# uuwee/Vulkan-PBR-Renderer

Hardware: AMD Instinct MI355X
Metric: IBL-prefilter Mtexels/s (specular prefilter all mips + irradiance; PBR-shaded Mpixels/s under extra.shade_c5 / extra.shade) (higher is better)
Workload: dtype f32; 1 GPU; C4: 4096x4096 specular prefilter (6 faces, 13 mips) + 128x128 irradiance from a 2048^2 HDR cube; env=procedural HDR cube 2048^2 x6 RGBA32F (seed 0x5eed0004, RGBE round-tripped), overlap=False, parallelism=single GPU

## Files before the change

include/pbr_kernels.h:

```cpp
#ifndef PBR_KERNELS_H
#define PBR_KERNELS_H

#include <stddef.h>
#include <stdint.h>

#ifdef __cplusplus
extern "C" {
#endif

enum {
    PBRK_OK = 0,
    PBRK_E_ARG = -1,
    PBRK_E_FORMAT = -2,
    PBRK_E_LAUNCH = -3
};

enum {
    PBRK_FMT_RG16F = 1,
    PBRK_FMT_RG32F = 2,
    PBRK_FMT_RGBA16F = 3,
    PBRK_FMT_RGBA32F = 4,
    PBRK_FMT_R32F = 5,
    PBRK_FMT_RGBA8UN = 6,
    PBRK_FMT_BGRA8UN = 7
// ... 41 lines not shown
size_t pbrk_cells_bytes(int n_src);
int pbrk_cells_build(const void* bordered_level, int n_src, void* cells, void* stream);
int pbrk_mc_filter(const void* src_bordered_level, const void* src_cells, int n_src, const void* table4, int n_entries,
                   float divisor, float alpha, void* out, int out_size,
                   int face0, int face1, int y0, int y1, void* stream);

int pbrk_mc_region_stats(unsigned long long* out2, int reset);
void pbrk_mc_set_kernels(int region, int lds);
int pbrk_mc_region_flag_stats(unsigned long long* out3);
int pbrk_mc_region_window_stats(unsigned long long* out1);
int pbrk_mc_region_skip_stats(unsigned long long* out3);
void pbrk_mc_set_absorb(int on);
void pbrk_mc_set_runs(int on);
void pbrk_mc_set_prologue(int lean);
int pbrk_mc_region_phase_stats(unsigned long long* out5);
int pbrk_mc_region_order(int face, int G, int k);
void pbrk_mc_set_launch_cut(int on);
int pbrk_mc_launch_cut(const float* weights, int n, unsigned min_bits, unsigned max_bits, int* cut4);
int pbrk_mc_launch_cut_slices(const float* weights, int n, int S, unsigned min_bits, unsigned max_bits, int* cut);
int pbrk_mc_launch_cut_stats(int* out6);
void pbrk_mc_set_tile32(int mode);
void pbrk_mc_set_fold(int on);
int pbrk_mc_last_fold(void);
void pbrk_mc_set_resident(int on);
int pbrk_mc_resident_stats(unsigned long long* out4);

typedef struct PbrkShadeArgs {
    int width, height;
    int x0, x1, y0, y1;
    const void* base_color;
    const void* normal;
    const void* orm;
    const void* emissive;
    const void* depth;
    const void* irradiance_bordered;
    int irradiance_size;
    const void* prefiltered_bordered;
    int prefiltered_size, prefiltered_levels;
    const void* lut;
    int lut_size;
    const void* irradiance_cells;
    const void* prefiltered_cells;
    int prefiltered_cells_first;
    const void* lut_cells;
    const void* sun_depth;
    int sun_depth_w, sun_depth_h;
// ... 150 lines not shown
```

vulkan-pbr-renderer_amd/csrc/k_mc_internal.h:

```cpp
#pragma once
#include <hip/hip_runtime.h>
#include "pbr_device.h"

struct McArgs {
    const float4* src; int n_src; unsigned src_bytes;
    const float4* cells; unsigned cells_bytes;
    const float4* tab; int n_tab;
    float divisor, alpha;
    float4* out; int size;
    int face0, y0, rows, tiles_x, tiles_per_face;
    int snap;
};

typedef unsigned int u32x3 __attribute__((ext_vector_type(3)));


__device__ __forceinline__ f3 tap_rgb(__amdgpu_buffer_rsrc_t rs, int voff, int soff) {
    u32x3 v = __builtin_amdgcn_raw_buffer_load_b96(rs, voff, soff, 0);
    return mk3(__uint_as_float(v.x), __uint_as_float(v.y), __uint_as_float(v.z));
}

typedef unsigned int u32x4c __attribute__((ext_vector_type(4)));
__device__ __forceinline__ f3 fetch_cells(__amdgpu_buffer_rsrc_t rc, int voff, float a, float b) {
    u32x4c A = __builtin_amdgcn_raw_buffer_load_b128(rc, voff, 0, 0);
// ... 44 lines not shown
    union { unsigned u; float f; } cm, cM, cW;
    cm.u = min_bits; cM.u = max_bits;
    const double m = (double)cm.f, M = (double)cM.f;
    int ncut = 0;
    for (int s = 0; s < S; ++s) {
        const double rhs = H[s] * m;
        if (!(rhs * 0x1p-25 >= 0x1p-100)) continue;
        int c = cut[s];
        for (int w = c - S; w > s; w -= S) {
            cW.u = wbits[w];
            const double lhs = (double)cW.f * M * 0x1p25 * (1.0 + 0x1p-10);
            if (!(lhs <= rhs)) break;
            c = w;
        }
        ncut += (cut[s] - c) / S;
        cut[s] = c;
    }
    return ncut;
}
__host__ __device__ inline int mc_launch_cut(const unsigned* wbits, int NW, const double* H, unsigned min_bits, unsigned max_bits, int* cut4) {
    return mc_launch_cut_s(wbits, NW, 4, H, min_bits, max_bits, cut4);
}

bool launch_mc_region(McArgs a, int nfaces, hipStream_t st);
bool launch_mc_resident(McArgs a, int nfaces, hipStream_t st);
extern int g_mc_region_mode, g_mc_lds_mode;
```

vulkan-pbr-renderer_amd/csrc/k_mc_region.hip:

```cpp
#include "pbr_device.h"
#include "pbr_kernels.h"
#include "k_mc_internal.h"

#include <stdlib.h>
#include <mutex>
#include <type_traits>

typedef float v4f __attribute__((ext_vector_type(4)));
typedef const __attribute__((address_space(4))) v4f* ctab_t;
typedef const __attribute__((address_space(3))) v4f* lds_v4f_p;
typedef const __attribute__((address_space(4))) unsigned* cu32_t;

#define REG_MAX_S 16
#ifndef MC_HEAD_FIRST_SUB
#define MC_HEAD_FIRST_SUB 1
#endif
#ifndef MC_HEAD_FIRST_G1
#define MC_HEAD_FIRST_G1 1
#endif
#ifndef MC_CERT_G1
#define MC_CERT_G1 1
#endif

#ifndef MC_TAP_JOIN_G1
#define MC_TAP_JOIN_G1 1
#endif

#ifndef MC_TILE32_SUB
#define MC_TILE32_SUB 1
#endif
#ifndef MC_TILE32_MIN_SIZE
#define MC_TILE32_MIN_SIZE 1024
#endif

struct RegArgs {
    McArgs a;
    int G;
    int RC;
    int NR;
    int NW;
    int expect[REG_MAX_S];
    int pole_row[2];
    const unsigned* tabmax;
    int cut;
    int absorb;
    unsigned long long* stats;
};

__device__ __forceinline__ void face_coords(int f, float x, float y, float z, float& sc, float& tc, float& ma) {
    switch (f) {
    case 0: sc = -z; tc = -y; ma = x; break;
    case 1: sc = z; tc = -y; ma = -x; break;
// ... 56 lines not shown
    unsigned long long inm = __builtin_amdgcn_ballot_w64(c1) & __builtin_amdgcn_ballot_w64(c2);
    if (inm == 0) return;
    if (!ACC && !SUB) { cnt += (unsigned)__builtin_popcountll(inm); return; }
    bool in = c1 && c2;
    const float h = __builtin_amdgcn_rcpf(ma) * V.half_n;
    const float u = fmaf(sc, h, V.off), v = fmaf(tc, h, V.off);
    if (SUB) {
        const bool c3 = u >= V.ulo, c4 = u < V.uhi, c5 = v >= V.vlo, c6 = v < V.vhi;
        inm &= __builtin_amdgcn_ballot_w64(c3) & __builtin_amdgcn_ballot_w64(c4) & __builtin_amdgcn_ballot_w64(c5) & __builtin_amdgcn_ballot_w64(c6);
        in = in && c3 && c4 && c5 && c6;
    }
    cnt += (unsigned)__builtin_popcountll(inm);
    if (ACC && in) tap_accumulate<RS>(e.w, u, v, V.lds_base, ar, ag, ab);
}

template <int RS, bool FOLD = false, bool JOIN = false>
__device__ __forceinline__ void certain_sample(const v4f e, const RegionView& V, float& ar, float& ag, float& ab) {
    float sc, tc, ma;
    to_face(e, V, sc, tc, ma);
    const float h = FOLD ? __builtin_amdgcn_rcpf(ma) : __builtin_amdgcn_rcpf(ma) * V.half_n;
    tap_accumulate<RS, JOIN>(e.w, fmaf(sc, h, V.off), fmaf(tc, h, V.off), V.lds_base, ar, ag, ab);
}

template <int RS, bool SUB, int CLS, bool ACC = true, bool FOLD = false, bool JOIN = false>
__device__ __forceinline__ void lane_sample(const v4f e, const RegionView& V, float& ar, float& ag, float& ab, unsigned& cnt) {
    float sc, tc, ma;
    to_face(e, V, sc, tc, ma);
    bool c1, c2;
    on_face<CLS>(sc, tc, FOLD ? ma * V.half_n : ma, c1, c2);
    bool in = c1 && c2;
    if (SUB && __builtin_amdgcn_ballot_w64(in) == 0ull) return;
    const float h = FOLD ? __builtin_amdgcn_rcpf(ma) : __builtin_amdgcn_rcpf(ma) * V.half_n;
    const float u = fmaf(sc, h, V.off), v = fmaf(tc, h, V.off);
    if (SUB) in = in && u >= V.ulo && u < V.uhi && v >= V.vlo && v < V.vhi;
    if (in) {
        cnt += 1u;
        if (ACC) tap_accumulate<RS, JOIN>(e.w, u, v, V.lds_base, ar, ag, ab);
    }
}

template <typename F>
__device__ __forceinline__ void each_sample(unsigned m, ctab_t tw, F&& f) {
    if (m == 0u) return;
    v4f e = tw[__builtin_ctz(m)];
    m &= m - 1u;
    while (m) {
        const v4f en = tw[__builtin_ctz(m)];
        m &= m - 1u;
        f(e);
        e = en;
    }
    f(e);
}

__device__ __forceinline__ float absorb_threshold(float wmax, float m) {
    const float t = wmax * m * 1.00000095367431640625f * 0x1p25f;
    return t < 0x1p-100f ? 0x1p-100f : t;
}

// ... 36 lines not shown
                    region_sample<RS, SUB, CLS, false>(tw[i0], V, ar, ag, ab, cnt);
                }
                continue;
            }
        }
        while (m) {
            const int i0 = __builtin_ctz(m);
            m &= m - 1u;
            const bool two = m != 0u;
            const int i1 = two ? __builtin_ctz(m) : i0;
            m &= m - 1u;
            const v4f e0 = tw[i0];
            const v4f e1 = tw[i1];
            if (CERT && ((c >> i0) & 1u)) certain_sample<RS>(e0, V, ar, ag, ab);
            else region_sample<RS, SUB, CLS>(e0, V, ar, ag, ab, cnt);
            if (two) {
                if (CERT && ((c >> i1) & 1u)) certain_sample<RS>(e1, V, ar, ag, ab);
                else region_sample<RS, SUB, CLS>(e1, V, ar, ag, ab, cnt);
            }
        }
    }
}

template <int RS, bool SUB, int CLS, int REG_S, bool CERT, bool LEAN, bool FOLD>
__device__ __forceinline__ void region_pass_runs(const RegionView& V, const unsigned* __restrict__ mwords, const unsigned* __restrict__ cwords, cu32_t wmg,
                                                 unsigned rbits, unsigned* skc, int NW, int s, unsigned long long wsel, ctab_t tab,
                                                 float& ar, float& ag, float& ab, unsigned& cnt) {
    const int wl = s + REG_S * (int)(threadIdx.x & 63);
    unsigned long long nz = __builtin_amdgcn_ballot_w64(wl < NW && mwords[wl] != 0u) & wsel;
    constexpr bool JOIN = FOLD && RS == 66 && !SUB && MC_TAP_JOIN_G1 != 0;
    auto tested = [&](const v4f e) { lane_sample<RS, SUB, CLS, true, FOLD, JOIN>(e, V, ar, ag, ab, cnt); };
    while (nz) {
        const int w = s + REG_S * (int)__builtin_ctzll(nz);
        nz &= nz - 1ull;
        const unsigned m = (unsigned)__builtin_amdgcn_readfirstlane((int)mwords[w]);
        unsigned c = CERT ? (unsigned)__builtin_amdgcn_readfirstlane((int)cwords[w]) : 0u;
        ctab_t tw = tab + (w << 5);
        const unsigned wb = rbits < 0x7f800000u ? (LEAN ? wmg[w] : (unsigned)__builtin_amdgcn_readfirstlane((int)cwords[NW + w])) : 0x7f800000u;
        if (wb < 0x7f800000u) {
            const float T = absorb_threshold(__uint_as_float(wb), __uint_as_float(rbits));
            if (__builtin_amdgcn_ballot_w64(!(ar >= T && ag >= T && ab >= T)) == 0ull) {
                if (!CERT) c = (unsigned)__builtin_amdgcn_readfirstlane((int)cwords[w]);
                cnt += (unsigned)__builtin_popcount(m & c);
                count_absorbed(skc, m, m & ~c);
                each_sample(m & ~c, tw, [&](const v4f e) { lane_sample<RS, SUB, CLS, false, FOLD>(e, V, ar, ag, ab, cnt); });
                continue;
            }
        }
        if (!CERT) { each_sample(m, tw, tested); continue; }
        cnt += (unsigned)__builtin_popcount(m & c);
        unsigned mc = m & c, mu = m & ~c;
        for (;;) {
            const unsigned below = mu ? (mu & (0u - mu)) - 1u : ~0u;
            each_sample(mc & below, tw, [&](const v4f e) { certain_sample<RS, FOLD, JOIN>(e, V, ar, ag, ab); });
            mc &= ~below;
            if (!mu) break;
            const int it = __builtin_ctz(mu);
            mu &= mu - 1u;
            tested(tw[it]);
        }
    }
}

template <bool LEAN, bool G1, bool TWO, bool PROOF, bool SOLE>
__device__ __forceinline__ void region_bin(unsigned* masks, unsigned* any, unsigned* dmax, int NR, int NW, int G, int RC, int n,
                                           f3 R, f3 T, f3 B, f3 Rc, f3 Tc, f3 Bc, ctab_t tab, int n_tab, int tid,
                                           unsigned* cmask, unsigned* wmax, int ntail, int lim, bool keep_cut, int head_end) {
    const float nf = (float)n;
    const float half_n = 0.5f * nf;
    const float off = 0.5f * nf + 0.5f;
    for (int k = tid; k < NR * NW + NR + 1 + ntail; k += 1024) masks[k] = 0u;
    __syncthreads();
    {
// ... 162 lines not shown
template <int REG_TX, int REG_S>
__device__ __forceinline__ void reduce_slices(float* red, int s, int t, float ar, float ag, float ab) {
    red[(s * REG_TX + t) * 3 + 0] = ar;
    red[(s * REG_TX + t) * 3 + 1] = ag;
    red[(s * REG_TX + t) * 3 + 2] = ab;
    __syncthreads();
    for (int stride = REG_S / 2; stride >= 1; stride >>= 1) {
        if (s < stride) {
            const int a2 = (s * REG_TX + t) * 3, b2 = ((s + stride) * REG_TX + t) * 3;
            red[a2 + 0] += red[b2 + 0];
            red[a2 + 1] += red[b2 + 1];
            red[a2 + 2] += red[b2 + 2];
        }
        __syncthreads();
    }
}

#ifdef PBR_MC_PHASE_STAMPS
#define STAMP() ((unsigned long long)__builtin_readcyclecounter())
#else
#define STAMP() 0ull
#endif

template <int RS, bool SUB, int TILE, bool RUNS = false, bool LEAN = false, bool FOLD = false>
__global__ __launch_bounds__(1024) __attribute__((amdgpu_waves_per_eu(8, 8))) void k_mc_region(const RegArgs q) {
    constexpr int REG_TX = TILE * TILE, REG_S = 1024 / REG_TX;
    static_assert(!FOLD || (RUNS && LEAN && RS != 18), "FOLD: the run loop of the lean 66^2 / 34^2 shapes only");
    constexpr bool CERT = SUB || (RUNS && (RS != 66 || MC_CERT_G1 != 0));
    constexpr bool ABS = RS == 66;
    const bool absorb_on = ABS && q.absorb;
    constexpr bool OWN_FIRST = ABS;
    constexpr bool TWO = RS == 66 && (SUB ? MC_HEAD_FIRST_SUB != 0 : MC_HEAD_FIRST_G1 != 0);
    const bool cut_on = TWO && LEAN && q.cut != 0;
    extern __shared__ __attribute__((aligned(16))) unsigned char smem_r[];
    float4* region = (float4*)smem_r;
    const unsigned lds_base = (unsigned)(unsigned long long)smem_r;
    unsigned* skc = (unsigned*)(smem_r + RS * RS * 16);
    unsigned* masks = skc + 4;
    unsigned* any = masks + q.NR * q.NW;
    unsigned* dmax = any + q.NR;
    unsigned* cmask = dmax + 1;
    unsigned* wmax = cmask + q.NW;
    unsigned* rmax = wmax + q.NW;
    const int ntail = (absorb_on && !LEAN) ? 2 * q.NW + q.NR : ((CERT || ABS) ? q.NW : 0);
    cu32_t wmg = (cu32_t)(unsigned long long)q.tabmax;
    [[maybe_unused]] const unsigned long long st0 = STAMP();
    const McArgs& p = q.a;
    const int tid = threadIdx.x;
    const int s = __builtin_amdgcn_readfirstlane(tid / REG_TX);
    const int t = tid % REG_TX;
// ... 9 lines not shown
    const f3 Rc = face_texel_dir(face, min(tx * TILE + TILE / 2, p.size - 1), min(p.y0 + ty * TILE + TILE / 2, p.y0 + p.rows - 1), p.size);
    const f3 Tc = tangent_of(Rc);
    const f3 Bc = cross3(Tc, Rc);

    const int n = p.n_src, nb = n + 2;
    const float nf = (float)n;
    const float half_n = 0.5f * nf;
    const float off = 0.5f * nf + 0.5f;
    ctab_t tab = (ctab_t)(unsigned long long)p.tab;
    const int NW = q.NW, NR = q.NR, G = q.G, RC = q.RC;

    if (ABS && tid < 4) skc[tid] = 0u;
    [[maybe_unused]] const unsigned long long st1 = STAMP();
    const int lim = cut_on ? (int)q.tabmax[NW + NR + ((tid >> 5) % REG_S)] << 5 : 0x7fffffff;
    region_bin<LEAN, !SUB, TWO, CERT || ABS, CERT && !SUB>(masks, any, dmax, NR, NW, G, RC, n, R, T, B, Rc, Tc, Bc, tab, p.n_tab, tid, (CERT || ABS) ? cmask : nullptr,
                                (absorb_on && !LEAN) ? wmax : nullptr, ntail, lim, cut_on && q.stats != nullptr, 32 * REG_S);
    [[maybe_unused]] unsigned long long st_stage = 0ull;
#ifdef PBR_MC_PHASE_STAMPS
    __syncthreads();
#endif
    [[maybe_unused]] const unsigned long long st2 = STAMP();

    float ar = 0.0f, ag = 0.0f, ab = 0.0f;
    unsigned cnt = cut_on ? cut_credit<REG_S, RUNS>((int)wmg[NW + NR + s], NW, p.n_tab) : 0u;
    if (q.stats) {
        __syncthreads();
        unsigned fl = 0, cfl = 0, cwd = 0;
        for (int k = tid; k < NR * NW; k += 1024) {
            const unsigned mk = masks[k];
            fl += __popc(mk);
            if (cut_on) {
                const int w = k % NW;
                if (w >= (int)q.tabmax[NW + NR + (w % REG_S)]) { cfl += __popc(mk); cwd += mk != 0u; masks[k] = 0u; }
            }
        }
        constexpr unsigned BLK = REG_TX / 256;
        if (fl) atomicAdd(&q.stats[2], (unsigned long long)(fl * BLK));
        if (cwd) { atomicAdd(&skc[0], (16u / REG_S) * cwd); atomicAdd(&skc[1], (16u / REG_S) * cfl); }
        if (tid == 0) { atomicAdd(&q.stats[3], (unsigned long long)p.n_tab * BLK); unsigned v = 0; for (int r = 0; r < NR; ++r) v += (any[r] & (TWO ? 0xffffu : ~0u)) != 0u; atomicAdd(&q.stats[4], (unsigned long long)(v * BLK));
                        if (CERT) { unsigned c = 0; for (int k = 0; k < NW; ++k) c += __popc(cmask[k]); atomicAdd(&q.stats[5], (unsigned long long)(c * BLK)); } }
    }
    auto visit = [&](const int r, const int ph) {
        const int f = r / (G * G);
        const int gy = (r / G) % G, gx = r % G;
        const int ox = gx * RC, oy = gy * RC;
        const int rcx = min(RC, n + 1 - ox), rcy = min(RC, n + 1 - oy);
        const float4* __restrict__ fsrc = p.src + ((size_t)f * nb + oy) * nb + ox;
        const unsigned long long sta = STAMP();
        unsigned rbits = 0x7f800000u;
        if (LEAN && RS == 66) stage_rows<RS>(region, fsrc, nb, rcx, rcy, tid);
        else stage_sweeps<RS, ABS && !LEAN>(region, fsrc, nb, rcx, rcy, tid, (absorb_on && !LEAN) ? &rmax[r] : nullptr);
        if (absorb_on && LEAN) rbits = wmg[NW + r];
        __syncthreads();
        if (absorb_on && !LEAN) rbits = (unsigned)__builtin_amdgcn_readfirstlane((int)rmax[r]);
        const unsigned long long stb = STAMP();
        RegionView V;
        V.lds_base = lds_base - (unsigned)(oy * RS + ox) * 16u;
        face_coords(f, B.x, B.y, B.z, V.Pb.x, V.Pb.y, V.Pb.z);
        face_coords(f, T.x, T.y, T.z, V.Pt.x, V.Pt.y, V.Pt.z);
        face_coords(f, R.x, R.y, R.z, V.Pr.x, V.Pr.y, V.Pr.z);
        V.half_n = half_n; V.off = off;
        if (FOLD) {
            V.Pb.x *= half_n; V.Pt.x *= half_n; V.Pr.x *= half_n;
            V.Pb.y *= half_n; V.Pt.y *= half_n; V.Pr.y *= half_n;
        }
        V.ulo = (float)ox; V.uhi = (float)(ox + rcx); V.vlo = (float)oy; V.vhi = (float)(oy + rcy);
        const unsigned* mw = masks + r * NW;
        unsigned* const sc = (ABS && q.stats) ? skc : nullptr;
        const unsigned long long wsel = TWO ? (ph ? ~1ull : 1ull) : ~0ull;
        const int w0 = (TWO && ph) ? s + REG_S : s, w1 = (TWO && !ph) ? min(NW, s + 1) : NW;
        auto pass = [&](auto cls) {
            constexpr int CLS = decltype(cls)::value;
            if (RUNS) region_pass_runs<RS, SUB, CLS, REG_S, CERT, LEAN, FOLD>(V, mw, cmask, wmg, rbits, sc, NW, s, wsel, tab, ar, ag, ab, cnt);
            else region_pass<RS, SUB, CLS, REG_S, CERT, LEAN>(V, mw, cmask, wmg, rbits, sc, NW, w0, w1, tab, ar, ag, ab, cnt);
        };
        switch (f >> 1) {
        case 0: pass(std::integral_constant<int, 0>()); break;
        case 1: pass(std::integral_constant<int, 1>()); break;
        default: pass(std::integral_constant<int, 2>()); break;
        }
        st_stage += stb - sta;
    };
    [[maybe_unused]] const unsigned long long st2b = STAMP();
    if (RUNS) __syncthreads();
    for (int kk = 0; kk < (TWO ? 2 * NR : NR); ++kk) {
        const int ph = TWO && kk >= NR, k = kk - (ph ? NR : 0);
        const int r = OWN_FIRST ? mc_region_visit(k, face * (G * G), G * G) : k;
        if (!RUNS) __syncthreads();
        const unsigned av = RUNS ? (unsigned)__builtin_amdgcn_readfirstlane((int)any[r]) : any[r];
        if ((TWO ? (av >> (8 * ph)) & 0xffu : av) == 0u) continue;
        if (RUNS) __syncthreads();
        visit(r, ph);
    }

    [[maybe_unused]] const unsigned long long st3 = STAMP();
    const bool healed = RUNS ? __builtin_amdgcn_ballot_w64(cnt != (unsigned)q.expect[s]) != 0ull : cnt != 64u * (unsigned)q.expect[s];
    if (healed) heal_slice<REG_S>(p, tab, NW, s, R, T, B, ar, ag, ab);
    if (q.stats && (tid & 63) == 0) {
        if (healed) atomicAdd(&q.stats[0], 1ull);
        atomicAdd(&q.stats[1], 1ull);
    }

    __syncthreads();
    if (absorb_on && q.stats && tid < 3 && skc[tid]) atomicAdd(&q.stats[6 + tid], (unsigned long long)skc[tid]);
    float* red = (float*)smem_r;
    reduce_slices<REG_TX, REG_S>(red, s, t, ar, ag, ab);
    int tid_o = tid, x_o, y_o;
    asm volatile("" : "+v"(tid_o));
    const int t_o = tid_o % REG_TX;
    texel_of_thread<TILE>(p, tx, ty, t_o, x_o, y_o);
    if (x_o < p.size && y_o < p.y0 + p.rows && s == 0) {
        float4 o;
        o.x = red[t_o * 3 + 0] / p.divisor; o.y = red[t_o * 3 + 1] / p.divisor; o.z = red[t_o * 3 + 2] / p.divisor; o.w = p.alpha;
        p.out[((size_t)face * p.size + y_o) * p.size + x_o] = o;
    }
#ifdef PBR_MC_PHASE_STAMPS
    if (q.stats && tid == 0) {
        atomicAdd(&q.stats[9], st1 - st0); atomicAdd(&q.stats[10], st2 - st1); atomicAdd(&q.stats[11], st_stage);
        atomicAdd(&q.stats[12], (st3 - st2b) - st_stage); atomicAdd(&q.stats[13], STAMP() - st3);
    }
#endif
}

#define RES_RS 18
// ... 149 lines not shown
extern "C" int pbrk_mc_region_order(int face, int G, int k) {
    if (face < 0 || face > 5 || G < 1 || k < 0 || k >= 6 * G * G) return -1;
    return mc_region_visit(k, face * (G * G), G * G);
}

static unsigned long long* g_reg_stats = nullptr;
#define REG_STATS_BYTES 160

static int read_stats(unsigned long long* out, int first_slot, int count) {
    if (!g_reg_stats || !out) return PBRK_E_ARG;
    return hipMemcpy(out, g_reg_stats + first_slot, (size_t)count * 8, hipMemcpyDeviceToHost) == hipSuccess ? PBRK_OK : PBRK_E_LAUNCH;
}
extern "C" int pbrk_mc_region_stats(unsigned long long* out2, int reset) {
    const int rc = read_stats(out2, 0, 2);
    if (rc != PBRK_OK) return rc;
    return (reset && hipMemset(g_reg_stats, 0, REG_STATS_BYTES) != hipSuccess) ? PBRK_E_LAUNCH : PBRK_OK;
}
extern "C" int pbrk_mc_region_skip_stats(unsigned long long* out3) { return read_stats(out3, 6, 3); }
extern "C" int pbrk_mc_region_window_stats(unsigned long long* out1) { return read_stats(out1, 5, 1); }
extern "C" int pbrk_mc_region_flag_stats(unsigned long long* out3) { return read_stats(out3, 2, 3); }
extern "C" int pbrk_mc_region_phase_stats(unsigned long long* out5) { return read_stats(out5, 9, 5); }

static int g_last_fold = 0;
template <int RS, bool SUB, int TILE, bool RUNS = false, bool LEAN = false, bool FOLD = false>
static void launch_region_t(const RegArgs& q, unsigned grid, size_t lds, hipStream_t st) {
    static bool attr_set = false;
    if (!attr_set) { (void)hipFuncSetAttribute((const void*)k_mc_region<RS, SUB, TILE, RUNS, LEAN, FOLD>, hipFuncAttributeMaxDynamicSharedMemorySize, 160 * 1024); attr_set = true; }
    g_last_fold = FOLD ? 1 : 0;
    hipLaunchKernelGGL((k_mc_region<RS, SUB, TILE, RUNS, LEAN, FOLD>), dim3(grid), dim3(1024), lds, st, q);
}

__global__ __launch_bounds__(256) void k_mc_prep(const float4* __restrict__ src, int n, int G, int RC, int NR,
                                                 const float4* __restrict__ tab, int n_tab, int NW, unsigned* __restrict__ out) {
    const int tid = threadIdx.x;
    if ((int)blockIdx.x >= NR) {
        const int w = ((int)blockIdx.x - NR) * 256 + tid;
        if (w >= NW) return;
        unsigned m = 0u;
        for (int i = w << 5; i < min((w << 5) + 32, n_tab); ++i) m = max(m, __float_as_uint(tab[i].w));
        out[w] = m;
        return;
    }
    __shared__ unsigned red, redlo;
    if (tid == 0) { red = 0u; redlo = 0xffffffffu; }
    __syncthreads();
    const int r = (int)blockIdx.x, nb = n + 2;
    const int f = r / (G * G), gy = (r / G) % G, gx = r % G;
    const int ox = gx * RC, oy = gy * RC;
    const int cols = min(RC, n + 1 - ox) + 1, rows = min(RC, n + 1 - oy) + 1;
    const float4* __restrict__ fsrc = src + ((size_t)f * nb + oy) * nb + ox;
    unsigned m = 0u, lo = 0xffffffffu;
    for (int k = tid; k < rows * cols; k += 256) {
// ... 4 lines not shown
    }
    atomicMax(&red, m);
    atomicMin(&redlo, lo);
    __syncthreads();
    if (tid == 0) { out[NW + r] = red; out[NW + NR + 4 + r] = redlo; }
}

__global__ __launch_bounds__(64) void k_mc_cut(const float4* __restrict__ tab, int n_tab, int NW, int NR, int S, unsigned* __restrict__ out) {
    __shared__ double H[4];
    const int tid = threadIdx.x;
    if (tid < 4) {
        double h = 0.0;
        if (tid < S && NW > S)
            for (int i = 0; i < 32; ++i) h += (double)tab[(tid << 5) + i].w;
        H[tid] = h;
    }
    __syncthreads();
    if (tid != 0) return;
    unsigned M = 0u, m = 0xffffffffu;
    for (int r = 0; r < NR; ++r) { M = max(M, out[NW + r]); m = min(m, out[NW + NR + 4 + r]); }
    int cut4[4];
    mc_launch_cut_s(out, NW, S, H, m, M, cut4);
    for (int s = 0; s < 4; ++s) out[NW + NR + s] = (unsigned)cut4[s % S];
}

extern "C" int pbrk_mc_launch_cut(const float* weights, int n, unsigned min_bits, unsigned max_bits, int* cut4) {
    return pbrk_mc_launch_cut_slices(weights, n, 4, min_bits, max_bits, cut4);
}
extern "C" int pbrk_mc_launch_cut_slices(const float* weights, int n, int S, unsigned min_bits, unsigned max_bits, int* cut4) {
    if (!weights || !cut4 || n < 1 || n > 8192 || (S != 1 && S != 2 && S != 4)) return -1;
    const int NW = (n + 31) / 32;
    unsigned wbits[256];
    for (int w = 0; w < NW; ++w) {
        unsigned m = 0u;
        for (int i = w << 5; i < (w << 5) + 32 && i < n; ++i) {
            union { float f; unsigned u; } c;
            c.f = weights[i];
            m = c.u > m ? c.u : m;
        }
        wbits[w] = m;
    }
    double H[4] = {0.0, 0.0, 0.0, 0.0};
    if (NW > S)
        for (int s = 0; s < S; ++s)
            for (int i = 0; i < 32; ++i) H[s] += (double)weights[(s << 5) + i];
    return mc_launch_cut_s(wbits, NW, S, H, min_bits, max_bits, cut4);
}

#define PREP_SLOTS 32
#define PREP_SLOT_WORDS 4096
#define PREP_MAX_DEVICES 16
struct PrepRing { unsigned* dev; hipEvent_t ev[PREP_SLOTS]; bool used[PREP_SLOTS]; unsigned next; };
static PrepRing g_prep[PREP_MAX_DEVICES];
static std::mutex g_prep_lock;

static unsigned* prep_acquire(hipStream_t st, int* slot_out) {
    hipStreamCaptureStatus cs = hipStreamCaptureStatusNone;
    if (hipStreamIsCapturing(st, &cs) != hipSuccess) { (void)hipGetLastError(); return nullptr; }
    if (cs != hipStreamCaptureStatusNone) return nullptr;
    int dev = 0;
    if (hipGetDevice(&dev) != hipSuccess || dev < 0 || dev >= PREP_MAX_DEVICES) return nullptr;
    PrepRing& R = g_prep[dev];
    if (!R.dev) {
        if (hipMalloc(&R.dev, (size_t)PREP_SLOTS * PREP_SLOT_WORDS * 4) != hipSuccess) { (void)hipGetLastError(); R.dev = nullptr; return nullptr; }
        for (int i = 0; i < PREP_SLOTS; ++i) {
            R.used[i] = false;
            if (hipEventCreateWithFlags(&R.ev[i], hipEventDisableTiming) != hipSuccess) { (void)hipGetLastError(); (void)hipFree(R.dev); R.dev = nullptr; return nullptr; }
        }
        R.next = 0;
    }
    const int slot = (int)(R.next++ % PREP_SLOTS);
    if (R.used[slot] && hipStreamWaitEvent(st, R.ev[slot], 0) != hipSuccess) { (void)hipGetLastError(); return nullptr; }
    *slot_out = slot;
    return R.dev + (size_t)slot * PREP_SLOT_WORDS;
}

int g_mc_region_mode = -1, g_mc_lds_mode = -1;
extern "C" void pbrk_mc_set_kernels(int region, int lds) { g_mc_region_mode = region; g_mc_lds_mode = lds; }
static int g_mc_absorb = 1;
extern "C" void pbrk_mc_set_absorb(int on) { g_mc_absorb = on ? 1 : 0; }
static int g_mc_runs = 1;
extern "C" void pbrk_mc_set_runs(int on) { g_mc_runs = on ? 1 : 0; }
static int g_mc_lean = 1;
extern "C" void pbrk_mc_set_prologue(int lean) { g_mc_lean = lean ? 1 : 0; }

static int g_mc_launch_cut = 1;
extern "C" void pbrk_mc_set_launch_cut(int on) { g_mc_launch_cut = on ? 1 : 0; }
static int g_mc_tile32 = -1;
extern "C" void pbrk_mc_set_tile32(int mode) { g_mc_tile32 = mode < 0 ? -1 : (mode ? 1 : 0); }
static int g_mc_fold = 1;
extern "C" void pbrk_mc_set_fold(int on) { g_mc_fold = on ? 1 : 0; }
extern "C" int pbrk_mc_last_fold(void) { return g_last_fold; }
static const unsigned* g_last_cut = nullptr;
static int g_last_cut_nw = 0, g_last_cut_s = 4;
extern "C" int pbrk_mc_launch_cut_stats(int* out6) {
    if (!out6) return PBRK_E_ARG;
    const int NW = g_last_cut_nw, S = g_last_cut_s;
    for (int j = 0; j < 4; ++j) { const int s = j % S; out6[j] = s >= NW ? s : s + S * ((NW - s + S - 1) / S); }
    out6[4] = NW; out6[5] = 0;
    if (!g_last_cut) return PBRK_OK;
    if (hipDeviceSynchronize() != hipSuccess) return PBRK_E_LAUNCH;
    int c[4];
    if (hipMemcpy(c, g_last_cut, 16, hipMemcpyDeviceToHost) != hipSuccess) return PBRK_E_LAUNCH;
    for (int s = 0; s < 4; ++s) { if (s < S) out6[5] += (out6[s] - c[s]) / S; out6[s] = c[s]; }
    return PBRK_OK;
}

template <int RS, bool SUB, int TILE, bool LEAN, bool HAS_RUNS = true>
static void launch_runs(const RegArgs& q, unsigned grid, size_t lds, hipStream_t st) {
    if constexpr (HAS_RUNS) {
        if (g_mc_runs && q.NW <= 64 * (1024 / (TILE * TILE))) {
            if constexpr (LEAN) {
                const int n = q.a.n_src;
                if (g_mc_fold && (n & (n - 1)) == 0) { launch_region_t<RS, SUB, TILE, true, true, true>(q, grid, lds, st); return; }
            }
            launch_region_t<RS, SUB, TILE, true, LEAN>(q, grid, lds, st);
            return;
        }
    }
    launch_region_t<RS, SUB, TILE, false, LEAN>(q, grid, lds, st);
}

template <bool LEAN>
static void launch_shape(int RS, int tile, const RegArgs& q, unsigned grid, size_t lds, hipStream_t st) {
    if (tile == 32) launch_runs<66, true, 32, LEAN>(q, grid, lds, st);
    else if (RS == 18) launch_runs<18, false, 16, LEAN, false>(q, grid, lds, st);
    else if (RS == 34) launch_runs<34, false, 16, LEAN>(q, grid, lds, st);
    else if (q.G == 1) launch_runs<66, false, 16, LEAN>(q, grid, lds, st);
    else launch_runs<66, true, 16, LEAN>(q, grid, lds, st);
}

static unsigned long long* reg_stats() {
    static int stats_on = -1;
    if (stats_on < 0) {
        const char* e = getenv("PBR_MC_STATS"); stats_on = e ? atoi(e) : 0;
        if (stats_on) { if (hipMalloc(&g_reg_stats, REG_STATS_BYTES) != hipSuccess) g_reg_stats = nullptr; else (void)hipMemset(g_reg_stats, 0, REG_STATS_BYTES); }
    }
// ... 31 lines not shown
    q.NW = (a.n_tab + 31) / 32;
    q.absorb = RS == 66 ? g_mc_absorb : 0;
    const size_t lds_fixed = (size_t)RS * RS * 16 + (4 + (size_t)q.NR * q.NW + q.NR + 1 + q.NW) * 4;
    size_t lds = lds_fixed + (q.absorb ? (size_t)(q.NW + q.NR) * 4 : 0);
    if (lds > 80 * 1024) { q.absorb = 0; lds = lds_fixed; }
    if (lds < (size_t)1024 * 3 * 4) lds = (size_t)1024 * 3 * 4;
    if (lds > 80 * 1024) return false;
    q.stats = reg_stats();
    const int tile = mc_tile32(a.n_src, a.n_tab, a.size) ? 32 : 16, nslices = 1024 / (tile * tile);
    for (int s = 0; s < REG_MAX_S; ++s) q.expect[s] = 0;
    for (int w = 0; w < q.NW; ++w) { int c = a.n_tab - w * 32; q.expect[w % nslices] += c > 32 ? 32 : c; }
    q.a.tiles_x = (a.size + tile - 1) / tile;
    const int tiles_y = (a.rows + tile - 1) / tile;
    q.a.tiles_per_face = q.a.tiles_x * tiles_y;
    pole_rows(a.size, a.y0, tile, tiles_y, q.pole_row);
    const unsigned grid = (unsigned)(q.a.tiles_per_face * nfaces);
    bool lean = g_mc_lean != 0;
    q.tabmax = nullptr;
    q.cut = 0;
    g_last_cut = nullptr; g_last_cut_nw = q.NW; g_last_cut_s = nslices;
    if (lean && q.absorb) {
        std::lock_guard<std::mutex> hold(g_prep_lock);
        int slot = -1;
        unsigned* scratch = q.NW + 2 * q.NR + 4 <= PREP_SLOT_WORDS ? prep_acquire(st, &slot) : nullptr;
        if (!scratch) lean = false;
        else {
            int dev = 0; (void)hipGetDevice(&dev);
            q.tabmax = scratch;
            hipLaunchKernelGGL(k_mc_prep, dim3((unsigned)(q.NR + (q.NW + 255) / 256)), dim3(256), 0, st, a.src, a.n_src, q.G, q.RC, q.NR, a.tab, a.n_tab, q.NW, scratch);
            const bool head_first = RS == 66 && (q.G == 1 ? MC_HEAD_FIRST_G1 != 0 : MC_HEAD_FIRST_SUB != 0);
            if (head_first && g_mc_launch_cut && q.NW > nslices) {
                hipLaunchKernelGGL(k_mc_cut, dim3(1), dim3(64), 0, st, a.tab, a.n_tab, q.NW, q.NR, nslices, scratch);
                q.cut = 1;
                g_last_cut = scratch + q.NW + q.NR;
            }
            launch_shape<true>(RS, tile, q, grid, lds, st);
            if (hipEventRecord(g_prep[dev].ev[slot], st) == hipSuccess) g_prep[dev].used[slot] = true;
            return true;
        }
    }
    if (lean) launch_shape<true>(RS, tile, q, grid, lds, st);
    else launch_shape<false>(RS, tile, q, grid, lds, st);
    return true;
}

#ifndef MC_RESIDENT_TILE8
#define MC_RESIDENT_TILE8 1
#endif
static int g_mc_resident = -1;
extern "C" void pbrk_mc_set_resident(int on) { g_mc_resident = on < 0 ? -1 : (on ? 1 : 0); }
extern "C" int pbrk_mc_resident_stats(unsigned long long* out4) { return read_stats(out4, 16, 4); }

template <int TILE, bool FOLD, bool STATS>
static void launch_resident_t(const ResArgs& g, unsigned grid, size_t lds, hipStream_t st) {
    hipLaunchKernelGGL((k_mc_resident<TILE, FOLD, STATS>), dim3(grid), dim3(1024), lds, st, g);
}
// ... 34 lines not shown
```

vulkan-pbr-renderer_amd/python/pbrhip/__init__.py:

```python
import ctypes as C
import os

import numpy as np

_PKG = os.path.dirname(os.path.abspath(__file__))
PKG_ROOT = os.path.dirname(os.path.dirname(_PKG))
REPO_ROOT = os.path.dirname(PKG_ROOT)
LIB_PATH = os.path.join(PKG_ROOT, "libgpu_hip.so")

(Format_Invalid, Format_R8UN, Format_RG8UN, Format_RGBA8UN, Format_BGRA8UN, Format_R16F, Format_RG16F, Format_RGB16F,
 Format_RGBA16F, Format_R32F, Format_RG32F, Format_RGB32F, Format_RGBA32F, Format_R8I, Format_R16I, Format_RG16I,
 Format_RGBA16I, Format_R32I, Format_RG32I, Format_RGB32I, Format_RGBA32I, Format_R64I, Format_D16UN,
 Format_D32F_Or_X8D24UN) = range(24)
Format_BC1_RGB_UN, Format_BC1_RGBA_UN, Format_BC3_RGBA_UN, Format_BC5_UN = 26, 27, 28, 29
BC_BLOCK_BYTES = {Format_BC1_RGB_UN: 8, Format_BC1_RGBA_UN: 8, Format_BC3_RGBA_UN: 16, Format_BC5_UN: 16}
PBRK_BC1_RGB, PBRK_BC1_RGBA, PBRK_BC3, PBRK_BC5 = 0, 1, 2, 3
PBR_DDS_FILE_MIPS = 1
PBR_DDS_MAX_LEVELS = 16
PBR_DDS_OUT_SAME, PBR_DDS_OUT_RGBA16F, PBR_DDS_OUT_BC6H_UF16 = 0, 1, 2
TextureFlag_StorageImage, TextureFlag_RenderTarget, TextureFlag_HasMipmaps, TextureFlag_Cubemap = 1, 2, 4, 8
BufferFlag_CPU, BufferFlag_GPU, BufferFlag_StorageBuffer = 1, 2, 4
Shade_IBL, Shade_LightShafts = 1, 2
Unit_Prefilter, Unit_Irradiance, Unit_BrdfLut = 0, 1, 2

# ... 263 lines not shown
    "pbrk_mc_set_kernels": (None, [C.c_int, C.c_int]), "pbrk_shade_set_fast": (None, [C.c_int]), "pbrk_shade_last_kernel": (C.c_int, []),
    "pbrk_border_build": (C.c_int, [VP, VP, C.c_int, C.c_int, VP]),
    "pbrk_border_build_range": (C.c_int, [VP, VP, C.c_int, C.c_int, C.c_int, C.c_int, VP]),
    "pbrk_debug_sample": (C.c_int, [C.c_int, VP, C.c_int, C.c_int, C.c_int, VP, C.c_int, VP, VP]),
    "pbrk_bloom_pass": (C.c_int, [VP, VP]),
    "pbrk_taa_resolve": (C.c_int, [VP, VP]), "pbrk_final_post_process": (C.c_int, [VP, VP]),
    "pbrk_lightgrid_sweep": (C.c_int, [VP, C.c_int, C.c_int, C.c_int, C.c_int, C.c_int, C.c_int, C.c_int, C.c_int, VP]),
    "pbrk_brdf_lut": (C.c_int, [VP, C.c_int, C.c_int, C.c_int, VP, VP, C.c_int, C.c_int, VP]),
    "pbrk_prefilter_copy": (C.c_int, [VP, C.c_int, VP, C.c_int, C.c_int, C.c_int, C.c_int, C.c_int, VP]),
    "pbrk_mc_filter": (C.c_int, [VP, VP, C.c_int, VP, C.c_int, C.c_float, C.c_float, VP, C.c_int, C.c_int, C.c_int, C.c_int, C.c_int, VP]),
    "pbrk_cells_bytes": (C.c_size_t, [C.c_int]), "pbrk_cells_build": (C.c_int, [VP, C.c_int, VP, VP]),
    "pbrk_shade": (C.c_int, [C.POINTER(PbrkShadeArgs), VP]),
    "pbrk_lightgrid_view": (C.c_int, [C.POINTER(PbrkGridViewArgs), VP]),
    "pbrk_mc_region_stats": (C.c_int, [C.POINTER(C.c_uint64), C.c_int]),
    "pbrk_mc_region_flag_stats": (C.c_int, [C.POINTER(C.c_uint64)]), "pbrk_mc_region_window_stats": (C.c_int, [C.POINTER(C.c_uint64)]),
    "pbrk_mc_region_skip_stats": (C.c_int, [C.POINTER(C.c_uint64)]), "pbrk_mc_set_absorb": (None, [C.c_int]),
    "pbrk_mc_set_runs": (None, [C.c_int]), "pbrk_mc_region_order": (C.c_int, [C.c_int, C.c_int, C.c_int]),
    "pbrk_mc_set_prologue": (None, [C.c_int]), "pbrk_mc_set_launch_cut": (None, [C.c_int]),
    "pbrk_mc_launch_cut": (C.c_int, [C.POINTER(C.c_float), C.c_int, C.c_uint, C.c_uint, C.POINTER(C.c_int)]),
    "pbrk_mc_launch_cut_stats": (C.c_int, [C.POINTER(C.c_int)]),
    "pbrk_mc_launch_cut_slices": (C.c_int, [C.POINTER(C.c_float), C.c_int, C.c_int, C.c_uint, C.c_uint, C.POINTER(C.c_int)]),
    "pbrk_mc_set_tile32": (None, [C.c_int]),
    "pbrk_mc_set_fold": (None, [C.c_int]), "pbrk_mc_last_fold": (C.c_int, []),
    "pbrk_mc_set_resident": (None, [C.c_int]), "pbrk_mc_resident_stats": (C.c_int, [C.POINTER(C.c_uint64)]),
    "pbrk_mc_region_phase_stats": (C.c_int, [C.POINTER(C.c_uint64)]),
    "pbrk_lut_cells_build": (C.c_int, [VP, C.c_int, VP, VP]),
    "pbrk_equirect_to_cube": (C.c_int, [VP, C.c_int, C.c_int, VP, C.c_int, VP]),
    "pbrk_raster_scratch_bytes": (C.c_size_t, [U32, C.c_int, C.c_int]),
    "pbrk_raster_setup": (C.c_int, [VP, VP]), "pbrk_raster_tiles": (C.c_int, [VP, VP]),
    "pbrk_geometry_scratch_bytes": (C.c_size_t, [U32, C.c_int, C.c_int]),
    "pbrk_geometry_setup": (C.c_int, [VP, VP]), "pbrk_geometry_tiles": (C.c_int, [VP, VP]),
    "pbrk_voxelize_scratch_bytes": (C.c_size_t, [U32, C.c_int, C.c_int]),
    "pbrk_voxelize_cover": (C.c_int, [VP, VP]), "pbrk_voxelize_resolve": (C.c_int, [VP, VP]),
    "pbrk_mip_chain_rgba8": (C.c_int, [VP, C.c_int, C.c_int, C.c_int, VP]),
    "pbrk_bc_decode": (C.c_int, [C.c_int, VP, C.c_int, C.c_int, VP, VP]),
    "pbrk_sh9_scratch_bytes": (C.c_size_t, [C.c_int]),
    "pbrk_sh9_project": (C.c_int, [VP, C.c_int, C.c_int, C.c_int, C.c_int, C.c_int, VP, VP, VP]),
    "pbrk_sh9_irradiance": (C.c_int, [VP, VP, C.c_int, C.c_int, C.c_int, C.c_int, C.c_int, VP]),
    "GPUX_OpProjectSH9": (None, [VP, TexP, U32, U32, U32, U32, U32, BufP, U32]),
    "GPUX_OpIrradianceFromSH9": (None, [VP, BufP, U32, TexP, U32]),
    "PBR_ProjectSH9": (C.c_int, [TexP, U32, C.POINTER(C.c_double)]), "PBR_GenIrradianceMapSH": (None, [TexP, U32, TexP]),
    "PBR_EvalSH9Irradiance": (None, [C.POINTER(C.c_double), C.POINTER(C.c_float), C.POINTER(C.c_float)]),
    "PBR_WriteSH9File": (C.c_int, [C.c_char_p, C.POINTER(C.c_double)]), "PBR_ReadSH9File": (C.c_int, [C.c_char_p, C.POINTER(C.c_double)]),
    "pbrk_bc6h_level_bytes": (C.c_uint64, [C.c_int, C.c_int, C.c_int]),
    "pbrk_bc6h_encode": (C.c_int, [VP, C.c_int, C.c_int, C.c_int, C.c_int, VP, VP]),
    "GPUX_OpEncodeBC6H": (None, [VP, TexP, U32, BufP, U32]), "GPUX_BC6HMipBytes": (C.c_uint64, [TexP, U32]),
# ... 344 lines not shown
```

vulkan-pbr-renderer_amd/python/pbrhip/mc.py:

```python
import contextlib
import ctypes as C
import hashlib

import numpy as np

import pbrhip

SWITCH_DEFAULTS = {"absorb": (1,), "runs": (1,), "prologue": (1,), "launch_cut": (1,), "tile32": (-1,), "fold": (1,), "kernels": (-1, -1)}


@contextlib.contextmanager
def switches(L, **named):
    unknown = set(named) - set(SWITCH_DEFAULTS)
    if unknown:
        raise TypeError(f"unknown switch {sorted(unknown)}: one of {sorted(SWITCH_DEFAULTS)}")
    for name, value in named.items():
        getattr(L, "pbrk_mc_set_" + name)(*(value if name == "kernels" else (value,)))
    try:
        yield
    finally:
        for name in named:
            getattr(L, "pbrk_mc_set_" + name)(*SWITCH_DEFAULTS[name])


_GROUPS = {
    "region": ("pbrk_mc_region_stats", C.c_uint64, 2, lambda a: {"healed": int(a[0]), "slices": int(a[1])}),
    "skip": ("pbrk_mc_region_skip_stats", C.c_uint64, 3, lambda a: {"abs_words": int(a[0]), "abs_samples": int(a[1]), "count_only": int(a[2])}),
    "flag": ("pbrk_mc_region_flag_stats", C.c_uint64, 3, lambda a: {"flags": int(a[0]), "flag_samples": int(a[1]), "visits": int(a[2])}),
    "window": ("pbrk_mc_region_window_stats", C.c_uint64, 1, lambda a: {"proved": int(a[0])}),
    "cut": ("pbrk_mc_launch_cut_stats", C.c_int, 6, lambda a: {"cut4": list(a)[:4], "nw": int(a[4]), "words_cut": int(a[5])}),
    "phase": ("pbrk_mc_region_phase_stats", C.c_uint64, 5, lambda a: {"phase": tuple(int(v) for v in a)}),
# ... 113 lines not shown
```

Measured before the change: 2928 Mtexels/s.

## Add count-free region kernel variant with monotone early exit of absorbed words

Adds a NET=false instantiation of the lean run-loop region kernel. It drops per-sample coverage counting and the heal pass, and recomputes the bitangent via a cross product to save registers. Using a per-slice monotone index computed in the cut kernel, it breaks out of the word loop once every lane is absorbed and the remaining table words have non-increasing max weights. The variant is chosen by default whenever stats are off. The trade is that the heal safety net is lost, so correctness rests on the absorb/monotone bound being exact.

Measured after the change: 3056 Mtexels/s, median of 6. 4.4% higher.

```diff
diff --git a/include/pbr_kernels.h b/include/pbr_kernels.h
--- a/include/pbr_kernels.h
+++ b/include/pbr_kernels.h
@@ -87,6 +87,9 @@
 void pbrk_mc_set_tile32(int mode);
 void pbrk_mc_set_fold(int on);
 int pbrk_mc_last_fold(void);
+void pbrk_mc_set_net(int mode);
+int pbrk_mc_last_net(void);
+int pbrk_mc_mono_slices(const float* weights, int n, int S, int* mono4);
 void pbrk_mc_set_resident(int on);
 int pbrk_mc_resident_stats(unsigned long long* out4);
 
diff --git a/vulkan-pbr-renderer_amd/csrc/k_mc_internal.h b/vulkan-pbr-renderer_amd/csrc/k_mc_internal.h
--- a/vulkan-pbr-renderer_amd/csrc/k_mc_internal.h
+++ b/vulkan-pbr-renderer_amd/csrc/k_mc_internal.h
@@ -90,6 +90,17 @@
     return mc_launch_cut_s(wbits, NW, 4, H, min_bits, max_bits, cut4);
 }
 
+__host__ __device__ inline void mc_mono_from(const unsigned* wbits, int NW, int S, int* mono) {
+    for (int s = 0; s < S; ++s) {
+        int k = s;
+        if (s < NW) {
+            k = s + S * ((NW - 1 - s) / S);
+            while (k - S >= s && wbits[k - S] >= wbits[k]) k -= S;
+        }
+        mono[s] = k;
+    }
+}
+
 bool launch_mc_region(McArgs a, int nfaces, hipStream_t st);
 bool launch_mc_resident(McArgs a, int nfaces, hipStream_t st);
 extern int g_mc_region_mode, g_mc_lds_mode;
diff --git a/vulkan-pbr-renderer_amd/csrc/k_mc_region.hip b/vulkan-pbr-renderer_amd/csrc/k_mc_region.hip
--- a/vulkan-pbr-renderer_amd/csrc/k_mc_region.hip
+++ b/vulkan-pbr-renderer_amd/csrc/k_mc_region.hip
@@ -28,6 +28,12 @@
 
 #ifndef MC_TILE32_SUB
 #define MC_TILE32_SUB 1
+#endif
+#ifndef MC_NET_OFF_34
+#define MC_NET_OFF_34 1
+#endif
+#ifndef MC_MONO_EXIT
+#define MC_MONO_EXIT 1
 #endif
 #ifndef MC_TILE32_MIN_SIZE
 #define MC_TILE32_MIN_SIZE 1024
@@ -130,7 +136,7 @@
     tap_accumulate<RS, JOIN>(e.w, fmaf(sc, h, V.off), fmaf(tc, h, V.off), V.lds_base, ar, ag, ab);
 }
 
-template <int RS, bool SUB, int CLS, bool ACC = true, bool FOLD = false, bool JOIN = false>
+template <int RS, bool SUB, int CLS, bool ACC = true, bool FOLD = false, bool JOIN = false, bool NET = true>
 __device__ __forceinline__ void lane_sample(const v4f e, const RegionView& V, float& ar, float& ag, float& ab, unsigned& cnt) {
     float sc, tc, ma;
     to_face(e, V, sc, tc, ma);
@@ -142,7 +148,7 @@
     const float u = fmaf(sc, h, V.off), v = fmaf(tc, h, V.off);
     if (SUB) in = in && u >= V.ulo && u < V.uhi && v >= V.vlo && v < V.vhi;
     if (in) {
-        cnt += 1u;
+        if (NET) cnt += 1u;
         if (ACC) tap_accumulate<RS, JOIN>(e.w, u, v, V.lds_base, ar, ag, ab);
     }
 }
@@ -225,14 +231,14 @@
     }
 }
 
-template <int RS, bool SUB, int CLS, int REG_S, bool CERT, bool LEAN, bool FOLD>
+template <int RS, bool SUB, int CLS, int REG_S, bool CERT, bool LEAN, bool FOLD, bool NET = true>
 __device__ __forceinline__ void region_pass_runs(const RegionView& V, const unsigned* __restrict__ mwords, const unsigned* __restrict__ cwords, cu32_t wmg,
                                                  unsigned rbits, unsigned* skc, int NW, int s, unsigned long long wsel, ctab_t tab,
-                                                 float& ar, float& ag, float& ab, unsigned& cnt) {
+                                                 float& ar, float& ag, float& ab, unsigned& cnt, const RegArgs& q) {
     const int wl = s + REG_S * (int)(threadIdx.x & 63);
     unsigned long long nz = __builtin_amdgcn_ballot_w64(wl < NW && mwords[wl] != 0u) & wsel;
     constexpr bool JOIN = FOLD && RS == 66 && !SUB && MC_TAP_JOIN_G1 != 0;
-    auto tested = [&](const v4f e) { lane_sample<RS, SUB, CLS, true, FOLD, JOIN>(e, V, ar, ag, ab, cnt); };
+    auto tested = [&](const v4f e) { lane_sample<RS, SUB, CLS, true, FOLD, JOIN, NET>(e, V, ar, ag, ab, cnt); };
     while (nz) {
         const int w = s + REG_S * (int)__builtin_ctzll(nz);
         nz &= nz - 1ull;
@@ -243,6 +249,17 @@
         if (wb < 0x7f800000u) {
             const float T = absorb_threshold(__uint_as_float(wb), __uint_as_float(rbits));
             if (__builtin_amdgcn_ballot_w64(!(ar >= T && ag >= T && ab >= T)) == 0ull) {
+                if (!NET) {
+                    count_absorbed(skc, m, 0u);
+                    if (MC_MONO_EXIT == 0 || !(q.cut & 2) || w < (int)wmg[NW + 2 * q.NR + 4 + s]) continue;
+                    if (skc)
+                        while (nz) {
+                            const int wr = s + REG_S * (int)__builtin_ctzll(nz);
+                            nz &= nz - 1ull;
+                            count_absorbed(skc, (unsigned)__builtin_amdgcn_readfirstlane((int)mwords[wr]), 0u);
+                        }
+                    break;
+                }
                 if (!CERT) c = (unsigned)__builtin_amdgcn_readfirstlane((int)cwords[w]);
                 cnt += (unsigned)__builtin_popcount(m & c);
                 count_absorbed(skc, m, m & ~c);
@@ -251,7 +268,7 @@
             }
         }
         if (!CERT) { each_sample(m, tw, tested); continue; }
-        cnt += (unsigned)__builtin_popcount(m & c);
+        if (NET) cnt += (unsigned)__builtin_popcount(m & c);
         unsigned mc = m & c, mu = m & ~c;
         for (;;) {
             const unsigned below = mu ? (mu & (0u - mu)) - 1u : ~0u;
@@ -460,10 +477,11 @@
 #define STAMP() 0ull
 #endif
 
-template <int RS, bool SUB, int TILE, bool RUNS = false, bool LEAN = false, bool FOLD = false>
+template <int RS, bool SUB, int TILE, bool RUNS = false, bool LEAN = false, bool FOLD = false, bool NET = true>
 __global__ __launch_bounds__(1024) __attribute__((amdgpu_waves_per_eu(8, 8))) void k_mc_region(const RegArgs q) {
     constexpr int REG_TX = TILE * TILE, REG_S = 1024 / REG_TX;
     static_assert(!FOLD || (RUNS && LEAN && RS != 18), "FOLD: the run loop of the lean 66^2 / 34^2 shapes only");
+    static_assert(NET || (RUNS && LEAN && RS != 18), "NET = false: the run loop of the lean 66^2 / 34^2 shapes only");
     constexpr bool CERT = SUB || (RUNS && (RS != 66 || MC_CERT_G1 != 0));
     constexpr bool ABS = RS == 66;
     const bool absorb_on = ABS && q.absorb;
@@ -519,7 +537,7 @@
     [[maybe_unused]] const unsigned long long st2 = STAMP();
 
     float ar = 0.0f, ag = 0.0f, ab = 0.0f;
-    unsigned cnt = cut_on ? cut_credit<REG_S, RUNS>((int)wmg[NW + NR + s], NW, p.n_tab) : 0u;
+    unsigned cnt = (NET && cut_on) ? cut_credit<REG_S, RUNS>((int)wmg[NW + NR + s], NW, p.n_tab) : 0u;
     if (q.stats) {
         __syncthreads();
         unsigned fl = 0, cfl = 0, cwd = 0;
@@ -553,7 +571,13 @@
         const unsigned long long stb = STAMP();
         RegionView V;
         V.lds_base = lds_base - (unsigned)(oy * RS + ox) * 16u;
-        face_coords(f, B.x, B.y, B.z, V.Pb.x, V.Pb.y, V.Pb.z);
+        f3 Bv = B;
+        if constexpr (!NET) {
+            f3 Tq = T;
+            asm volatile("" : "+v"(Tq.x), "+v"(Tq.y), "+v"(Tq.z));
+            Bv = cross3(Tq, R);
+        }
+        face_coords(f, Bv.x, Bv.y, Bv.z, V.Pb.x, V.Pb.y, V.Pb.z);
         face_coords(f, T.x, T.y, T.z, V.Pt.x, V.Pt.y, V.Pt.z);
         face_coords(f, R.x, R.y, R.z, V.Pr.x, V.Pr.y, V.Pr.z);
         V.half_n = half_n; V.off = off;
@@ -568,7 +592,7 @@
         const int w0 = (TWO && ph) ? s + REG_S : s, w1 = (TWO && !ph) ? min(NW, s + 1) : NW;
         auto pass = [&](auto cls) {
             constexpr int CLS = decltype(cls)::value;
-            if (RUNS) region_pass_runs<RS, SUB, CLS, REG_S, CERT, LEAN, FOLD>(V, mw, cmask, wmg, rbits, sc, NW, s, wsel, tab, ar, ag, ab, cnt);
+            if (RUNS) region_pass_runs<RS, SUB, CLS, REG_S, CERT, LEAN, FOLD, NET>(V, mw, cmask, wmg, rbits, sc, NW, s, wsel, tab, ar, ag, ab, cnt, q);
             else region_pass<RS, SUB, CLS, REG_S, CERT, LEAN>(V, mw, cmask, wmg, rbits, sc, NW, w0, w1, tab, ar, ag, ab, cnt);
         };
         switch (f >> 1) {
@@ -591,12 +615,14 @@
     }
 
     [[maybe_unused]] const unsigned long long st3 = STAMP();
-    const bool healed = RUNS ? __builtin_amdgcn_ballot_w64(cnt != (unsigned)q.expect[s]) != 0ull : cnt != 64u * (unsigned)q.expect[s];
-    if (healed) heal_slice<REG_S>(p, tab, NW, s, R, T, B, ar, ag, ab);
-    if (q.stats && (tid & 63) == 0) {
-        if (healed) atomicAdd(&q.stats[0], 1ull);
-        atomicAdd(&q.stats[1], 1ull);
-    }
+    if constexpr (NET) {
+        const bool healed = RUNS ? __builtin_amdgcn_ballot_w64(cnt != (unsigned)q.expect[s]) != 0ull : cnt != 64u * (unsigned)q.expect[s];
+        if (healed) heal_slice<REG_S>(p, tab, NW, s, R, T, B, ar, ag, ab);
+        if (q.stats && (tid & 63) == 0) {
+            if (healed) atomicAdd(&q.stats[0], 1ull);
+            atomicAdd(&q.stats[1], 1ull);
+        }
+    } else if (q.stats && (tid & 63) == 0) atomicAdd(&q.stats[1], 1ull);
 
     __syncthreads();
     if (absorb_on && q.stats && tid < 3 && skc[tid]) atomicAdd(&q.stats[6 + tid], (unsigned long long)skc[tid]);
@@ -792,12 +818,14 @@
 extern "C" int pbrk_mc_region_phase_stats(unsigned long long* out5) { return read_stats(out5, 9, 5); }
 
 static int g_last_fold = 0;
-template <int RS, bool SUB, int TILE, bool RUNS = false, bool LEAN = false, bool FOLD = false>
+static int g_last_net = 1;
+template <int RS, bool SUB, int TILE, bool RUNS = false, bool LEAN = false, bool FOLD = false, bool NET = true>
 static void launch_region_t(const RegArgs& q, unsigned grid, size_t lds, hipStream_t st) {
     static bool attr_set = false;
-    if (!attr_set) { (void)hipFuncSetAttribute((const void*)k_mc_region<RS, SUB, TILE, RUNS, LEAN, FOLD>, hipFuncAttributeMaxDynamicSharedMemorySize, 160 * 1024); attr_set = true; }
+    if (!attr_set) { (void)hipFuncSetAttribute((const void*)k_mc_region<RS, SUB, TILE, RUNS, LEAN, FOLD, NET>, hipFuncAttributeMaxDynamicSharedMemorySize, 160 * 1024); attr_set = true; }
     g_last_fold = FOLD ? 1 : 0;
-    hipLaunchKernelGGL((k_mc_region<RS, SUB, TILE, RUNS, LEAN, FOLD>), dim3(grid), dim3(1024), lds, st, q);
+    g_last_net = NET ? 1 : 0;
+    hipLaunchKernelGGL((k_mc_region<RS, SUB, TILE, RUNS, LEAN, FOLD, NET>), dim3(grid), dim3(1024), lds, st, q);
 }
 
 __global__ __launch_bounds__(256) void k_mc_prep(const float4* __restrict__ src, int n, int G, int RC, int NR,
@@ -848,6 +876,9 @@
     int cut4[4];
     mc_launch_cut_s(out, NW, S, H, m, M, cut4);
     for (int s = 0; s < 4; ++s) out[NW + NR + s] = (unsigned)cut4[s % S];
+    int mono4[4];
+    mc_mono_from(out, NW, S, mono4);
+    for (int s = 0; s < 4; ++s) out[NW + 2 * NR + 4 + s] = (unsigned)mono4[s % S];
 }
 
 extern "C" int pbrk_mc_launch_cut(const float* weights, int n, unsigned min_bits, unsigned max_bits, int* cut4) {
@@ -871,6 +902,23 @@
         for (int s = 0; s < S; ++s)
             for (int i = 0; i < 32; ++i) H[s] += (double)weights[(s << 5) + i];
     return mc_launch_cut_s(wbits, NW, S, H, min_bits, max_bits, cut4);
+}
+
+extern "C" int pbrk_mc_mono_slices(const float* weights, int n, int S, int* mono4) {
+    if (!weights || !mono4 || n < 1 || n > 8192 || (S != 1 && S != 2 && S != 4)) return -1;
+    const int NW = (n + 31) / 32;
+    unsigned wbits[256];
+    for (int w = 0; w < NW; ++w) {
+        unsigned m = 0u;
+        for (int i = w << 5; i < (w << 5) + 32 && i < n; ++i) {
+            union { float f; unsigned u; } c;
+            c.f = weights[i];
+            m = c.u > m ? c.u : m;
+        }
+        wbits[w] = m;
+    }
+    mc_mono_from(wbits, NW, S, mono4);
+    return 0;
 }
 
 #define PREP_SLOTS 32
@@ -917,6 +965,9 @@
 static int g_mc_fold = 1;
 extern "C" void pbrk_mc_set_fold(int on) { g_mc_fold = on ? 1 : 0; }
 extern "C" int pbrk_mc_last_fold(void) { return g_last_fold; }
+static int g_mc_net = -1;
+extern "C" void pbrk_mc_set_net(int mode) { g_mc_net = mode < 0 ? -1 : (mode ? 1 : 0); }
+extern "C" int pbrk_mc_last_net(void) { return g_last_net; }
 static const unsigned* g_last_cut = nullptr;
 static int g_last_cut_nw = 0, g_last_cut_s = 4;
 extern "C" int pbrk_mc_launch_cut_stats(int* out6) {
@@ -938,7 +989,15 @@
         if (g_mc_runs && q.NW <= 64 * (1024 / (TILE * TILE))) {
             if constexpr (LEAN) {
                 const int n = q.a.n_src;
-                if (g_mc_fold && (n & (n - 1)) == 0) { launch_region_t<RS, SUB, TILE, true, true, true>(q, grid, lds, st); return; }
+                const bool fold = g_mc_fold && (n & (n - 1)) == 0;
+                if constexpr (RS != 34 || MC_NET_OFF_34 != 0) {
+                    if (!(g_mc_net < 0 ? q.stats != nullptr : g_mc_net != 0)) {
+                        if (fold) launch_region_t<RS, SUB, TILE, true, true, true, false>(q, grid, lds, st);
+                        else launch_region_t<RS, SUB, TILE, true, true, false, false>(q, grid, lds, st);
+                        return;
+                    }
+                }
+                if (fold) { launch_region_t<RS, SUB, TILE, true, true, true>(q, grid, lds, st); return; }
             }
             launch_region_t<RS, SUB, TILE, true, LEAN>(q, grid, lds, st);
             return;
@@ -1016,7 +1075,7 @@
     if (lean && q.absorb) {
         std::lock_guard<std::mutex> hold(g_prep_lock);
         int slot = -1;
-        unsigned* scratch = q.NW + 2 * q.NR + 4 <= PREP_SLOT_WORDS ? prep_acquire(st, &slot) : nullptr;
+        unsigned* scratch = q.NW + 2 * q.NR + 8 <= PREP_SLOT_WORDS ? prep_acquire(st, &slot) : nullptr;
         if (!scratch) lean = false;
         else {
             int dev = 0; (void)hipGetDevice(&dev);
@@ -1025,7 +1084,7 @@
             const bool head_first = RS == 66 && (q.G == 1 ? MC_HEAD_FIRST_G1 != 0 : MC_HEAD_FIRST_SUB != 0);
             if (head_first && g_mc_launch_cut && q.NW > nslices) {
                 hipLaunchKernelGGL(k_mc_cut, dim3(1), dim3(64), 0, st, a.tab, a.n_tab, q.NW, q.NR, nslices, scratch);
-                q.cut = 1;
+                q.cut = 3;
                 g_last_cut = scratch + q.NW + q.NR;
             }
             launch_shape<true>(RS, tile, q, grid, lds, st);
diff --git a/vulkan-pbr-renderer_amd/python/pbrhip/__init__.py b/vulkan-pbr-renderer_amd/python/pbrhip/__init__.py
--- a/vulkan-pbr-renderer_amd/python/pbrhip/__init__.py
+++ b/vulkan-pbr-renderer_amd/python/pbrhip/__init__.py
@@ -309,6 +309,8 @@
     "pbrk_mc_launch_cut_slices": (C.c_int, [C.POINTER(C.c_float), C.c_int, C.c_int, C.c_uint, C.c_uint, C.POINTER(C.c_int)]),
     "pbrk_mc_set_tile32": (None, [C.c_int]),
     "pbrk_mc_set_fold": (None, [C.c_int]), "pbrk_mc_last_fold": (C.c_int, []),
+    "pbrk_mc_set_net": (None, [C.c_int]), "pbrk_mc_last_net": (C.c_int, []),
+    "pbrk_mc_mono_slices": (C.c_int, [C.POINTER(C.c_float), C.c_int, C.c_int, C.POINTER(C.c_int)]),
     "pbrk_mc_set_resident": (None, [C.c_int]), "pbrk_mc_resident_stats": (C.c_int, [C.POINTER(C.c_uint64)]),
     "pbrk_mc_region_phase_stats": (C.c_int, [C.POINTER(C.c_uint64)]),
     "pbrk_lut_cells_build": (C.c_int, [VP, C.c_int, VP, VP]),
diff --git a/vulkan-pbr-renderer_amd/python/pbrhip/mc.py b/vulkan-pbr-renderer_amd/python/pbrhip/mc.py
--- a/vulkan-pbr-renderer_amd/python/pbrhip/mc.py
+++ b/vulkan-pbr-renderer_amd/python/pbrhip/mc.py
@@ -6,7 +6,8 @@
 
 import pbrhip
 
-SWITCH_DEFAULTS = {"absorb": (1,), "runs": (1,), "prologue": (1,), "launch_cut": (1,), "tile32": (-1,), "fold": (1,), "kernels": (-1, -1)}
+SWITCH_DEFAULTS = {"absorb": (1,), "runs": (1,), "prologue": (1,), "launch_cut": (1,), "tile32": (-1,), "fold": (1,), "net": (-1,),
+                   "kernels": (-1, -1)}
 
 
 @contextlib.contextmanager
```
